# orybkin/video-gcp

Measured on AMD Instinct MI355X. Metric: predicted frames/sec, 64x64x3 seq_len=80 gcp_tree (posterior forward + all loss terms, model(inputs) and model.loss() of train.py:157-159, batch-stat BatchNorm), higher is better.
Workload: dtype f32 (encoder / decoder convs and the tree GEMMs from 512 rows: split-f16 MFMA with f32 accumulate, f32-equivalent; everything else exact f32 MFMA)

## Files before the change

### include/gcpx.h

```cpp
#ifndef GCPX_H
#define GCPX_H

#include <stdint.h>

#ifdef __cplusplus
extern "C" {
#endif

#define GCPX_VERSION 1

typedef enum gcpx_status {
    GCPX_OK = 0,
    GCPX_ERR_INVALID_ARG = -1,
    GCPX_ERR_UNSUPPORTED = -2,
    GCPX_ERR_HIP = -3,
    GCPX_ERR_COMM = -4
} gcpx_status;

typedef enum gcpx_act { GCPX_ACT_NONE = 0, GCPX_ACT_LRELU = 1, GCPX_ACT_TANH = 2 } gcpx_act;

int gcpx_version(void);
const char* gcpx_last_error(void);
int gcpx_conv_grid(void);

// ... 23 lines not shown
    int32_t Hin, Win;
    int32_t Hout, Wout;
    int32_t Cin;
    int32_t Cout;
    int32_t out_pitch;
    int32_t upsample;
    int32_t out_act;
    int32_t head_mode;
    const float* wpk;
    const float* bias;
    float* out;
    float* images;
    float* stats_partial;
    const int32_t* raw_row_map;
    const int32_t* src_row_map;
    const int32_t* src_row_frames;
    int32_t n_src_rows;
    int32_t w_split_log2;
    const void* wpk_split;
    const int32_t* w_split_log2_dev;
    int32_t split_layout;
    int32_t nll_rows;
    const float* nll_target;
    float* nll_partial;
    const float* nll_row_weight;
    float nll_scale;
    int32_t _pad3;
    float* images_rows;
    int64_t images_rows_dup;
    const float* bwd_r;
    const float *bwd_scale, *bwd_shift, *bwd_mean, *bwd_rstd;
    const float* addend;
    int32_t addend_frame_div;
    int32_t _pad4;
} gcpx_conv_args;

typedef enum gcpx_split_layout { GCPX_SPLIT_PLAIN = 0, GCPX_SPLIT_ROWFOLD = 1, GCPX_SPLIT_HEAD32 = 2, GCPX_SPLIT_ROWFOLD16 = 3,
                                 GCPX_SPLIT_LOWRES = 4 } gcpx_split_layout;

int gcpx_conv3x3(const gcpx_conv_args* a, void* stream);
int gcpx_conv3x3_grid(const gcpx_conv_args* a);
int gcpx_conv3x3_lowres_supported(const gcpx_conv_args* a);
int gcpx_conv4x4s2(const gcpx_conv_args* a, void* stream);
int gcpx_conv4x4s2_grid(void);
int gcpx_conv4x4s2_image(const float* x, const float* wpk, const float* bias, float* out,
                         int32_t F, int32_t Hin, int32_t Win, int32_t Cout, int32_t out_act, void* stream);

int gcpx_bn_finalize(const float* partial, int32_t n_partial, int32_t pitch, int32_t C, double count,
                     const float* gamma, const float* beta, float eps, float* scale, float* shift,
                     float* running_mean, float* running_var, float momentum, float* mean_out, float* rstd_out,
                     void* stream);
int gcpx_randn(float* out, int64_t n, uint64_t* state, void* stream);
int gcpx_bn_fold(const float* running_mean, const float* running_var, const float* gamma, const float* beta,
                 float eps, int32_t C, float* scale, float* shift, void* stream);

typedef struct gcpx_row_src {
    const float* ptr;
    const int32_t* rowidx;
    const float* scale;
    const float* shiftv;
    int64_t sb, sr;
    int32_t width;
    int32_t shift;
    int32_t act;
    int32_t cmod;
} gcpx_row_src;

typedef enum gcpx_gemm_epi {
    GCPX_EPI_NONE = 0,
    GCPX_EPI_LRELU = 1,
    GCPX_EPI_LSTM = 2,
    GCPX_EPI_GAUSS_SAMPLE = 3
} gcpx_gemm_epi;

struct gcpx_lstm_bwd_args;
// ... 552 lines not shown
```

### video-gcp_amd/csrc/conv3x3_split.hip

```cpp
#include "common.h"
#include "split_mfma.h"

#include <cstdlib>
#include <type_traits>

namespace {

struct SplitUpCfg {
    static constexpr int RW = 18, RH = 6, LW = 10, LH = 4, CC = 16, KS = 5;
    static constexpr int RAW_BYTES = LH * LW * CC * 4;
    static constexpr int PLANE_BYTES = RH * RW * 32;
    static constexpr int WAVE_BYTES = RAW_BYTES + 2 * PLANE_BYTES;
    static constexpr int NS = (LH * LW * 4 + 63) / 64;
    static constexpr int W_CHUNK_BYTES = KS * 2 * 1024;
    static int lds_bytes(int nchunk) { return nchunk * W_CHUNK_BYTES + 8 * WAVE_BYTES + 8 * 2 * 16 * 4; }
};

__global__ void __launch_bounds__(512, 2) conv3x3_up16_split_kernel(const gcpx_conv_args a, const int items_per_wave,
                                                                    const int nitems) {
    using Cfg = SplitUpCfg;
    constexpr int RW = Cfg::RW, RH = Cfg::RH, LW = Cfg::LW, LH = Cfg::LH, CC = Cfg::CC, NS = Cfg::NS, KS = Cfg::KS;
    extern __shared__ float4 smem4[];
    const int nchunk = a.Cin / CC;
    const char* wl = reinterpret_cast<const char*>(smem4);
// ... 1389 lines not shown

int gcpx_launch_up32_split(const gcpx_conv_args* a, hipStream_t stream, int which, int grid) {
    if (a->split_layout == GCPX_SPLIT_LOWRES) return gcpx_launch_lowres(a, stream, grid);
    if (which == 0) return launch_up32_split<2, 1>(a, stream, grid);
    if (which == 1) return launch_up32_split<2, 2>(a, stream, grid);
    return launch_up32_split<4, 2>(a, stream, grid);
}

int gcpx_launch_up16_fold(const gcpx_conv_args* a, hipStream_t stream, int grid) {
    using Cfg = FoldCfg;
    GCPX_CHECK_ARG(a->Cin == 32 && a->Cout == 16 && a->Hin % Cfg::R == 0 && a->Hout == 2 * a->Hin && a->Wout == 2 * a->Win && a->Wout % 16 == 0,
                   "row-folded block: 32 -> 16 channels, Hin a multiple of 4, output width a multiple of 16");
    GCPX_CHECK_ARG(a->src[0].C % 4 == 0 && (a->nsrc == 1 ? a->src[0].C == 32 : a->src[0].C + a->src[1].C == 32), "source channels");
    static const bool prio = getenv("GCPX_FOLD_NOPRIO") == nullptr;
    auto kern = prio ? conv3x3_up16_fold_kernel<true> : conv3x3_up16_fold_kernel<false>;
    static bool attr_set = false;
    if (!attr_set) {
        for (auto k : {conv3x3_up16_fold_kernel<true>, conv3x3_up16_fold_kernel<false>}) {
            hipError_t e = hipFuncSetAttribute(reinterpret_cast<const void*>(k), hipFuncAttributeMaxDynamicSharedMemorySize, Cfg::LDS_BYTES);
            if (e != hipSuccess) {
                gcpx_set_error("conv3x3 row-folded up16: hipFuncSetAttribute(%d B LDS): %s", Cfg::LDS_BYTES, hipGetErrorString(e));
                return GCPX_ERR_HIP;
            }
        }
        attr_set = true;
    }
    const int nitems = a->F * (a->Hin / Cfg::R) * (a->Wout / 16);
    const int ipw = (nitems + grid * 8 - 1) / (grid * 8);
    hipLaunchKernelGGL(kern, dim3(grid), dim3(512), Cfg::LDS_BYTES, stream, *a, ipw, nitems);
    GCPX_CHECK_LAUNCH();
    return GCPX_OK;
}

int gcpx_launch_up16_fold16(const gcpx_conv_args* a, hipStream_t stream, int grid) {
    using Cfg = Fold16Cfg;
    GCPX_CHECK_ARG(a->Cin == 16 && a->Cout == 16 && a->nsrc == 1 && a->src[0].C == 16 && a->Hin % Cfg::R == 0 && a->Hout == 2 * a->Hin &&
                   a->Wout == 2 * a->Win && a->Wout % 16 == 0,
                   "row-folded 16-channel block: one 16-channel source, 16 output channels, Hin a multiple of 4, output width a multiple of 16");
    GCPX_CHECK_ARG(!a->addend || (a->addend_frame_div > 0 && a->F % a->addend_frame_div == 0),
                   "row-folded 16-channel block: F must be a multiple of addend_frame_div (items are walked sequence by sequence)");
    auto kern = conv3x3_up16_fold16_kernel;
    static bool attr_set = false;
    if (!attr_set) {
        hipError_t e = hipFuncSetAttribute(reinterpret_cast<const void*>(kern), hipFuncAttributeMaxDynamicSharedMemorySize, Cfg::LDS_BYTES);
        if (e != hipSuccess) {
            gcpx_set_error("conv3x3 row-folded up16 (16 channels): hipFuncSetAttribute(%d B LDS): %s", Cfg::LDS_BYTES, hipGetErrorString(e));
            return GCPX_ERR_HIP;
        }
        attr_set = true;
    }
    const int nitems = a->F * (a->Hin / Cfg::R) * (a->Wout / 16);
    const int ipw = (nitems + grid * 8 - 1) / (grid * 8);
    hipLaunchKernelGGL(kern, dim3(grid), dim3(512), Cfg::LDS_BYTES, stream, *a, ipw, nitems);
    GCPX_CHECK_LAUNCH();
    return GCPX_OK;
}

extern "C" int gcpx_fold_upsample_weights(const float* w, int32_t Cout, int32_t Cin, float* out, void* stream_) {
    GCPX_CHECK_ARG(w && out && Cout > 0 && Cin > 0, "bad arguments");
    const int n = 24 * Cout * Cin;
    hipLaunchKernelGGL(fold_up_weights_kernel, dim3((n + 255) / 256), dim3(256), 0, reinterpret_cast<hipStream_t>(stream_), w, Cout, Cin, out);
    GCPX_CHECK_LAUNCH();
    return GCPX_OK;
}

int gcpx_launch_wave_split(const gcpx_conv_args* a, hipStream_t stream, int ct, int depth) {
    const int nchunk = a->Cin / 16;
    if (ct == 1) {
// ... 11 lines not shown
```

### video-gcp_amd/packing.py

```python
import torch

_LANE = torch.arange(64)
_LI = _LANE % 16
_LQ = _LANE // 16


def _pad_rows(w, rows):
    if w.shape[0] == rows:
        return w
    pad = torch.zeros((rows - w.shape[0],) + tuple(w.shape[1:]), dtype=w.dtype, device=w.device)
    return torch.cat([w, pad], 0)


def pack_gemm(w):
    N, K = w.shape
    assert K % 16 == 0, (N, K)
    NT = (N + 15) // 16
    w = _pad_rows(w, NT * 16)
    dev = w.device
    kg = torch.arange(K // 16, device=dev)[:, None, None, None]
    nt = torch.arange(NT, device=dev)[None, :, None, None]
    li = _LI.to(dev)[None, None, :, None]
    lq = _LQ.to(dev)[None, None, :, None]
    s = torch.arange(4, device=dev)[None, None, None, :]
# ... 236 lines not shown


def bilinear_x2_matrix(n, dtype=torch.float64):
    U = torch.zeros(2 * n, n, dtype=dtype)
    for h in range(2 * n):
        s = h // 2
        s0, s1, w0 = (s, min(s + 1, n - 1), 0.75) if h % 2 else (max(s - 1, 0), s, 0.25)
        U[h, s0] += w0
        U[h, s1] += 1.0 - w0
    return U


def lowres_up_reference(x, w, b):
    x, w = x.double(), w.double()
    Fr, _, H, W = x.shape
    cout = w.shape[0]
    Uy, Ux = bilinear_x2_matrix(H), bilinear_x2_matrix(W)
    out = torch.zeros(Fr, cout, 2 * H, 2 * W, dtype=torch.float64)
    for ty in range(3):
        z = torch.zeros(Fr, cout, H, 2 * W, dtype=torch.float64)
        for tx in range(3):
            y = torch.einsum("oc,fchw->fohw", w[:, :, ty, tx], x)
            yx = torch.einsum("fohw,pw->fohp", y, Ux)
            lo, hi = max(0, 1 - tx), min(2 * W, 2 * W + 1 - tx)
            z[..., lo:hi] += yx[..., lo + tx - 1:hi + tx - 1]
        zy = torch.einsum("qh,fohp->foqp", Uy, z)
        lo, hi = max(0, 1 - ty), min(2 * H, 2 * H + 1 - ty)
        out[:, :, lo:hi] += zy[:, :, lo + ty - 1:hi + ty - 1]
    if b is not None:
        out += b.double()[None, :, None, None]
    return out


def conv3x3_split32_index(shape, offset):
    n = 1
    for d in shape:
        n *= d
    ids = (torch.arange(n, dtype=torch.float64) + (offset + 1)).view(shape)
    return (conv3x3_split32_gather(ids).reshape(-1) - 1).to(torch.int32)


def head32_slot(c, i, n_mix=10):
    g, h, r = i // 8, (i // 4) % 2, i % 4
    if c < 3:
        m, p = 2 * c + g // 2, 4 * (g % 2) + r
        return 8 * (2 * m + h) + p if m < 5 else -1
    u = 4 * g + r
    return dlm_log_scale_slot(1 + u % 2, 2 * (u // 2) + h, n_mix) if u < 10 else -1


def head32_gather(w, perm):
    assert w.shape[1] == 16 and w.shape[0] == 100
    dev = w.device
    chan = torch.tensor([[perm[head32_slot(c, i)] if head32_slot(c, i) >= 0 else -1 for i in range(32)] for c in range(4)], device=dev)
    wz = torch.cat([w.reshape(100, 16, 9), torch.zeros((1, 16, 9), dtype=w.dtype, device=dev)], 0)
    chan = torch.where(chan >= 0, chan, torch.full_like(chan, 100))
    tap = torch.arange(9, device=dev)[:, None, None, None]
    ct = torch.arange(4, device=dev)[None, :, None, None]
    lane = torch.arange(64, device=dev)[None, None, :, None]
    el = torch.arange(8, device=dev)[None, None, None, :]
    return wz[chan[ct, lane % 32], (lane // 32) * 8 + el, tap].contiguous()


def pack_head32_split(w, perm):
    w1, w2, e = split_f16(head32_gather(w, perm))
    return torch.stack([w1, w2], 2).contiguous().view(torch.int16), e
# ... 39 lines not shown
def pack_conv3x3_fold(w):
    w1, w2, e = split_f16(conv3x3_fold_gather(fold_up_weights(w)))
    return torch.stack([w1, w2], 1).contiguous().view(torch.int16), e


def conv3x3_fold_index():
    ids = torch.arange(24 * 16 * 32, dtype=torch.float64).view(24, 16, 32)
    return conv3x3_fold_gather(ids).reshape(-1).to(torch.int32)


def conv3x3_fold16_gather(fw, cbase=0):
    assert fw.shape[0] == 24 and fw.shape[1] == 16 and fw.shape[2] >= cbase + 16
    dev = fw.device
    bases = [py * 9 + dyl * 3 for py in range(2) for dyl in range(3)] + [18, 21]
    fz = torch.cat([fw, torch.zeros((1,) + tuple(fw.shape[1:]), dtype=fw.dtype, device=dev)], 0)
    li, lq = _LI.to(dev)[:, None], _LQ.to(dev)[:, None]
    el = torch.arange(8, device=dev)[None, :]
    frags = []
    for b in bases:
        for kind in range(2):
            tset = (b + lq // 2) if kind == 0 else torch.where(lq // 2 == 0, torch.full_like(lq, b + 2), torch.full_like(lq, 24))
            frags.append(fz[tset, li, cbase + 8 * (lq % 2) + el])
    return torch.stack(frags, 0).contiguous()


def pack_conv3x3_fold16(w, cbase=0):
    w1, w2, e = split_f16(conv3x3_fold16_gather(fold_up_weights(w), cbase))
    return torch.stack([w1, w2], 1).contiguous().view(torch.int16), e


def conv3x3_fold16_index(cin, cbase):
    ids = (torch.arange(24 * 16 * cin, dtype=torch.float64) + 1).view(24, 16, cin)
    return (conv3x3_fold16_gather(ids, cbase).reshape(-1) - 1).to(torch.int32)


def lstm_gate_interleave(w_ih, w_hh, b_ih, b_hh):
    H = w_hh.shape[1]
    w = torch.cat([w_ih, w_hh], dim=1)
    K = w.shape[1]
    w = w.view(4, H, K).permute(1, 0, 2).reshape(4 * H, K)
    b = (b_ih + b_hh).view(4, H).t().reshape(4 * H)
    return w.contiguous(), b.contiguous()


def unpack_conv4x4(wpk, cin, cout):
    dev = wpk.device
    wpk = wpk.reshape(16, cin // 16, cout // 16, 64, 4)
    w = torch.zeros((cout, cin, 16), dtype=wpk.dtype, device=dev)
    tap = torch.arange(16, device=dev)[:, None, None, None, None]
    cg = torch.arange(cin // 16, device=dev)[None, :, None, None, None]
    ct = torch.arange(cout // 16, device=dev)[None, None, :, None, None]
    li = _LI.to(dev)[None, None, None, :, None]
    lq = _LQ.to(dev)[None, None, None, :, None]
    s = torch.arange(4, device=dev)[None, None, None, None, :]
    w[(ct * 16 + li).expand_as(wpk), (cg * 16 + lq * 4 + s).expand_as(wpk), tap.expand_as(wpk)] = wpk
    return w.reshape(cout, cin, 4, 4)


def encoder_frames_unsupported(hp):
    if hp.input_nc != 3:
        return f"input_nc = {hp.input_nc}: 3 is built"
    if hp.img_sz not in (32, 64):
        return f"img_sz = {hp.img_sz}: 32 and 64 are built"
    if hp.ngf != 16:
        return f"ngf = {hp.ngf}: 16 is built"
    if hp.nz_enc <= 0 or hp.nz_enc % 16 or hp.nz_enc > 256:
# ... 69 lines not shown
```

### video-gcp_amd/runtime.py

```python
import ctypes as C
import os

_HERE = os.path.dirname(os.path.abspath(__file__))
LIB_PATH = os.path.join(_HERE, "libgcpx.so")

ACT_NONE, ACT_LRELU, ACT_TANH = 0, 1, 2
HEAD_RAW, HEAD_DLM_MEAN, HEAD_DLM_BOTH, HEAD_TANH_NCHW, HEAD_DLM_NLL, HEAD_DLM_NLL_GRAD = 0, 1, 2, 3, 4, 5
SPLIT_PLAIN, SPLIT_ROWFOLD, SPLIT_HEAD32, SPLIT_ROWFOLD16, SPLIT_LOWRES = 0, 1, 2, 3, 4
EPI_NONE, EPI_LRELU, EPI_LSTM, EPI_GAUSS_SAMPLE = 0, 1, 2, 3
GEMM_FORM_TILE, GEMM_FORM_SPLIT_K, GEMM_FORM_SPLIT_F16, GEMM_FORM_PLANES = 0, 1, 2, 3
MLP_PLAIN, MLP_GAUSS, MLP_TANH = 0, 1, 2

vp = C.c_void_p
i32 = C.c_int32
i64 = C.c_int64


class ConvSrc(C.Structure):
    _fields_ = [("ptr", vp), ("scale", vp), ("shift", vp), ("C", i32), ("frame_div", i32), ("act", i32), ("_pad", i32)]


class ConvArgs(C.Structure):
    _fields_ = [("src", ConvSrc * 2), ("nsrc", i32), ("F", i32), ("Hin", i32), ("Win", i32), ("Hout", i32),
                ("Wout", i32), ("Cin", i32), ("Cout", i32), ("out_pitch", i32), ("upsample", i32), ("out_act", i32),
                ("head_mode", i32), ("wpk", vp), ("bias", vp), ("out", vp), ("images", vp), ("stats_partial", vp),
                ("raw_row_map", vp), ("src_row_map", vp), ("src_row_frames", vp), ("n_src_rows", i32), ("w_split_log2", i32), ("wpk_split", vp), ("w_split_log2_dev", vp),
                ("split_layout", i32), ("nll_rows", i32), ("nll_target", vp), ("nll_partial", vp), ("nll_row_weight", vp),
                ("nll_scale", C.c_float), ("_pad3", i32), ("images_rows", vp), ("images_rows_dup", i64), ("bwd_r", vp), ("bwd_scale", vp), ("bwd_shift", vp), ("bwd_mean", vp),
                ("bwd_rstd", vp), ("addend", vp), ("addend_frame_div", i32), ("_pad4", i32)]


class LossArgs(C.Structure):
    _fields_ = [("nll_bt", vp), ("pad_mask", vp), ("kl_b", vp), ("len_logits", vp), ("end_ind", vp), ("existence", vp),
                ("leave", vp), ("regressed_state", vp), ("state_target", vp), ("seq_len", vp), ("out", vp),
                ("B", i32), ("T", i32), ("N", i32), ("state_dim", i32), ("w_rec", C.c_float), ("w_kl", C.c_float),
                ("w_len", C.c_float), ("w_exist", C.c_float), ("w_state", C.c_float), ("total_div", C.c_float),
                ("action_pred", vp), ("action_seq", vp), ("inv_t0", vp), ("cost_pred", vp), ("cost_target", vp),
                ("n_actions", i32), ("w_action", C.c_float), ("w_cost", C.c_float), ("state_mask", vp), ("w_kl_dev", vp)]


class RowSrc(C.Structure):
    _fields_ = [("ptr", vp), ("rowidx", vp), ("scale", vp), ("shiftv", vp), ("sb", i64), ("sr", i64),
                ("width", i32), ("shift", i32), ("act", i32), ("cmod", i32)]


class GemmArgs(C.Structure):
    _fields_ = [("src", RowSrc * 6), ("nsrc", i32), ("M", i32), ("N", i32), ("K", i32), ("rpb", i32),
                ("wpk", vp), ("bias", vp), ("out", vp), ("ob", i64), ("orow", i64), ("epi", i32), ("nbatch", i32),
                ("stats_partial", vp), ("c_prev", vp), ("c_prev_stride", i64), ("h_out", vp), ("c_out", vp),
                ("hb", i64), ("hrow", i64), ("h_copy", vp), ("z_src_off", i64), ("z_w_off", i64),
                ("z_bias_off", i64), ("z_out_off", i64), ("gates_out", vp),
                ("wpk_split", vp), ("w_split_log2_dev", vp), ("w_split_log2", i32), ("_pad_split", i32),
                ("x_planes", vp), ("x_exp", vp), ("x_planes_bytes", i64), ("lstm_bwd", vp)]


class MlpArgs(C.Structure):
    _fields_ = [("src", RowSrc * 6), ("nsrc", i32), ("M", i32), ("rpb", i32), ("in_dim", i32), ("mid", i32),
                ("n_mid", i32), ("out_dim", i32), ("w_in", vp), ("b_in", vp), ("w_mid", vp), ("b_mid", vp),
                ("gn_gamma", vp), ("gn_beta", vp), ("w_out", vp), ("b_out", vp), ("gn_eps", C.c_float),
                ("lrelu_slope", C.c_float), ("epi", i32), ("out_split", i32), ("out", vp), ("ob", i64), ("orow", i64),
                ("oblk", i64), ("eps", vp), ("eb", i64), ("erow", i64), ("z", vp), ("zb", i64), ("zrow", i64), ("save", vp)]

# ... 40 lines not shown
class ActBwdArgs(C.Structure):
    _fields_ = [("da", vp), ("add", vp), ("r", vp), ("scale", vp), ("shift", vp), ("mean", vp), ("rstd", vp), ("dy", vp),
                ("stats_partial", vp), ("ldc", i64), ("c_off", i32), ("up", i32), ("fsum", i32), ("act", i32), ("F", i32),
                ("H", i32), ("W", i32), ("C", i32)]


class PanelTile(C.Structure):
    _fields_ = [("kind", i32), ("src", i32), ("index", i32), ("length", i32), ("flags", i32), ("nb", i32), ("nf", i32),
                ("h", i32), ("w", i32), ("tile_w", i32), ("n0", i32), ("n_b", i32), ("n_f", i32), ("r0", i32), ("r_b", i32),
                ("r_f", i32), ("c0", i32), ("c_b", i32), ("c_f", i32), ("index_off", i32), ("index_stride", i32),
                ("index_count", i32), ("fill", C.c_float), ("_pad", i32), ("off", i64), ("s_b", i64), ("s_f", i64), ("s_c", i64),
                ("s_y", i64)]


class TrajLayer(C.Structure):
    _fields_ = [("states", vp), ("s_n", i64), ("s_p", i64), ("s_d", i64), ("len", vp), ("dim_t", vp), ("color", C.c_float * 3),
                ("len_i64", i32), ("K", i32), ("P", i32)]


PANEL_MAX_SRCS = 16
PANEL_IMAGE, PANEL_GREY, PANEL_GREY_ADD, PANEL_FILL = 0, 1, 2, 3
PANEL_RESCALE, PANEL_LENGTH_STRICT, PANEL_INDEX_FRAME, PANEL_INDEX_I64, PANEL_LENGTH_I64 = 1, 2, 4, 8, 16

WG_ROWS, WG_CONV1D, WG_CONV3X3, WG_CONV4X4S2 = 0, 1, 2, 3
WMAP_LINEAR, WMAP_CONV, WMAP_CONVT = 0, 1, 2

SYMBOLS = [
    ("gcpx_version", C.c_int, []),
    ("gcpx_last_error", C.c_char_p, []),
    ("gcpx_conv_grid", C.c_int, []),
    ("gcpx_conv3x3", C.c_int, [C.POINTER(ConvArgs), vp]),
    ("gcpx_conv3x3_grid", C.c_int, [C.POINTER(ConvArgs)]),
    ("gcpx_conv3x3_lowres_supported", C.c_int, [C.POINTER(ConvArgs)]),
    ("gcpx_conv4x4s2", C.c_int, [C.POINTER(ConvArgs), vp]),
    ("gcpx_conv4x4s2_grid", C.c_int, []),
    ("gcpx_conv4x4s2_image", C.c_int, [vp, vp, vp, vp, i32, i32, i32, i32, i32, vp]),
    ("gcpx_bn_finalize", C.c_int, [vp, i32, i32, i32, C.c_double, vp, vp, C.c_float, vp, vp, vp, vp, C.c_float, vp, vp, vp]),
    ("gcpx_bn_fold", C.c_int, [vp, vp, vp, vp, C.c_float, i32, vp, vp, vp]),
    ("gcpx_randn", C.c_int, [vp, i64, vp, vp]),
    ("gcpx_gemm", C.c_int, [C.POINTER(GemmArgs), vp]),
    ("gcpx_gemm_row_blocks", C.c_int, [i32, i32]),
    ("gcpx_gemm_form", C.c_int, [C.POINTER(GemmArgs), vp]),
    ("gcpx_gemm_planes_workspace", C.c_int, [i32, i32, i32, vp, vp]),
    ("gcpx_mlp", C.c_int, [C.POINTER(MlpArgs), vp]),
    ("gcpx_balanced_binding", C.c_int, [vp, i32, i32, i32, vp, vp, vp, vp, vp, vp, vp]),
    ("gcpx_dlm_nll", C.c_int, [vp, vp, vp, vp, i32, i32, i32, i32, vp]),
    ("gcpx_gauss_nll", C.c_int, [vp, vp, vp, vp, i32, i32, vp]),
    ("gcpx_kl_gauss", C.c_int, [vp, vp, i32, i32, i32, i64, i64, C.c_float, vp, i64, vp, vp]),
    ("gcpx_gauss_sample", C.c_int, [vp, i64, i64, vp, i64, i64, vp, i64, i64, i32, i32, i32, vp]),
    ("gcpx_seq_index", C.c_int, [vp, i32, i32, vp, vp, vp]),
    ("gcpx_fill_zero", C.c_int, [vp, i64, vp]),
    ("gcpx_copy_rows", C.c_int, [vp, vp, i32, i32, i64, i64, i64, vp]),
    ("gcpx_loss_combine", C.c_int, [C.POINTER(LossArgs), vp]),
    ("gcpx_loss_pre", C.c_int, [C.POINTER(LossArgs), vp, vp, i32, i32, i64, i64, C.c_float, vp, i64, vp, vp]),
    ("gcpx_loss_final", C.c_int, [C.POINTER(LossArgs), vp]),
    ("gcpx_gather_rows", C.c_int, [vp, vp, vp, i32, i32, i32, i32, i64, vp]),
    ("gcpx_gather_rows_rest", C.c_int, [vp, vp, vp, i32, i32, i32, i32, i64, vp, vp]),
    ("gcpx_compact_index", C.c_int, [vp, i32, i32, i32, vp, vp]),
    ("gcpx_seq_pairs", C.c_int, [vp, vp, vp, vp, i32, i32, i32, vp]),
    ("gcpx_rollout_cost", C.c_int, [vp, i64, vp, vp, i64, vp, i32, i32, i32, i32, i32, C.c_float, vp]),
    ("gcpx_masked_row_sum", C.c_int, [vp, vp, vp, i32, i32, vp]),
    ("gcpx_wgrad", C.c_int, [C.POINTER(WgradArgs), vp]),
    ("gcpx_wgrad_classify", C.c_int, [C.POINTER(WgradArgs), i32, C.POINTER(C.c_int32), C.POINTER(C.c_int32)]),
    ("gcpx_wgrad_group", C.c_int, [vp, vp, i32, i32, i32, vp]),
    ("gcpx_wgrad_conv3x3", C.c_int, [vp, i32, vp, i32, i32, i32, i32, i32, vp, i32, vp]),
    ("gcpx_wgrad_conv3x3_split", C.c_int, [vp, i32, vp, i32, i32, i32, i32, i32, vp, i32, vp]),
# ... 164 lines not shown
```

### video-gcp_amd/weights.py

```python
import ctypes as C
import os
from contextlib import contextmanager

import torch

from . import packing as pk
from . import runtime as rt
from .hparams import GCPHParams
from .params import init_params, encoder_layers, encoder_skip_layers, decoder_layers
from .plan_ops import _addr


class WeightsMixin:

    def _flatten_params(self, params):
        off, self._poff = 0, {}
        for k, v in params.items():
            self._poff[k] = (off, tuple(v.shape))
            off += (v.numel() + 3) // 4 * 4
        self.theta = torch.zeros(off, dtype=torch.float32, device=self.device)
        self.sd = {}
        for k, v in params.items():
            o, shp = self._poff[k]
            view = self.theta[o:o + v.numel()].view(shp)
            view.copy_(v)
            self.sd[k] = view

    def _pack_predictor(self, prefix, out_dim):
        sd = self._psd
        mid = sd[f"{prefix}.input.linear.weight"].shape[0]
        n_mid = 0
        while f"{prefix}.pyramid-{n_mid}.linear.weight" in sd:
            n_mid += 1
        out_pad = (out_dim + 15) // 16 * 16
        w_in = sd[f"{prefix}.input.linear.weight"]
        k_raw = w_in.shape[1]
        if k_raw % 16:
            w_in = torch.cat([w_in, torch.zeros((mid, -k_raw % 16), dtype=w_in.dtype, device=w_in.device)], 1)
        d = dict(mid=mid, n_mid=n_mid, out_dim=out_dim, in_dim=w_in.shape[1], in_dim_raw=k_raw)
        d["w_in"] = pk.pack_gemm(w_in)
        d["b_in"] = sd[f"{prefix}.input.linear.bias"].contiguous()
        if n_mid:
            d["w_mid"] = torch.stack([pk.pack_gemm(sd[f"{prefix}.pyramid-{i}.linear.weight"]) for i in range(n_mid)]).contiguous()
# ... 29 lines not shown
                if self.split_f16 and skip_idx >= 0 and c_prev == 16 and c_skip == 16 and os.environ.get("GCPX_NO_SKIP_HOIST") is None:
                    hoist16.add(f"dec.{name}")
            elif cout == 16:
                todo.append((f"dec.{name}", f"decoder.net.{name}.conv.weight", None))
            elif cout in (32, 64) and (c_prev + c_skip) % 32 == 0:
                todo.append((f"dec.{name}", f"decoder.net.{name}.conv.weight", "tiled32"))
        for name, cin, cout, norm in self._enc_layers[1:]:
            if cin == 16 or cin % 32 == 0:
                todo.append((f"enc.{name}", f"encoder.net.{name}.conv.weight", "enc4x4"))
        for name, key, perm in todo:
            off, shp = self._poff[key]
            d = {}
            if perm == "enc4x4":
                idx = pk.conv4x4_split_index(shp, off).to(self.device)
            elif perm == "rowfold":
                d["fold"] = torch.zeros(24 * shp[0] * shp[1], dtype=torch.float32, device=self.device)
                d["fold_src"] = (off, shp[0], shp[1])
                idx = pk.conv3x3_fold_index().to(self.device)
            elif perm == "tiled32":
                idx = pk.conv3x3_split32_index(shp, off).to(self.device)
            elif isinstance(perm, tuple) and perm[0] == "head32":
                idx = pk.head32_index(shp, off, perm[1]).to(self.device)
            else:
                idx = pk.conv3x3_split_index(shp, off, perm).to(self.device)
            d.update(idx=idx, out=torch.zeros(2 * idx.numel(), dtype=torch.int16, device=self.device),
                     log2=torch.zeros(1, dtype=torch.int32, device=self.device))
            self.pk_split[name] = d
            if perm == "rowfold" and name in hoist16:
                for tag, cbase in (("f16a", 0), ("f16b", 16)):
                    i16 = pk.conv3x3_fold16_index(shp[1], cbase).to(self.device)
                    self.pk_split[f"{name}.{tag}"] = dict(fold=d["fold"], fold16=True, idx=i16,
                                                          out=torch.zeros(2 * i16.numel(), dtype=torch.int16, device=self.device),
                                                          log2=torch.zeros(1, dtype=torch.int32, device=self.device))
        self.repack_split()

    def repack_split(self, stream=None):
        st = stream if stream is not None else torch.cuda.current_stream(self.device).cuda_stream
        if not self.pk_split:
            return
        tab = self._split_tab
        key = (self.theta.data_ptr(),) + tuple((d["out"].data_ptr(), d["idx"].data_ptr()) for d in self.pk_split.values())
        if tab is None or tab[2] != key:
            descs = []
            for name, d in self.pk_split.items():
                src = d["fold"] if "fold" in d else self.theta
                e = rt.SplitPackDesc()
                e.src, e.idx, e.out, e.log2_out, e.n = src.data_ptr(), d["idx"].data_ptr(), d["out"].data_ptr(), d["log2"].data_ptr(), d["idx"].numel()
                descs.append(e)
            arr = (rt.SplitPackDesc * len(descs))(*descs)
            dev = torch.frombuffer(bytearray(bytes(arr)), dtype=torch.uint8).to(self.device)
            tab = self._split_tab = (dev, len(descs), key, torch.zeros(len(descs), dtype=torch.int32, device=self.device))
        for name, d in self.pk_split.items():
            if "fold_src" in d:
                off, cout, cin = d["fold_src"]
                rt.check(self.lib.gcpx_fold_upsample_weights(self.theta.data_ptr() + 4 * off, cout, cin, d["fold"].data_ptr(), st), "fold_upsample_weights")
        rt.check(self.lib.gcpx_split_pack_group2(tab[0].data_ptr(), tab[1], tab[3].data_ptr(), st), "split_pack_group2")

    def _pack_gemm_split(self):
        self._gsplit = {}
        self._merge_side_rows = int(os.environ.get("GCPX_MERGE_SIDE_ROWS", "512")) or (1 << 60)
        pr = int(os.environ.get("GCPX_GEMM_PLANES_ROWS", "512"))
        self._planes_min_rows = pr if pr > 0 else 1 << 60
        if not self.split_f16:
            return
        for name, W in self.pk.items():
            if not (isinstance(W, dict) and name.startswith("tree")):
                continue
            for key, wpk in W.items():
                if not (key.endswith(".w") and (key.startswith("lstm") or key == "proj.w")):
                    continue
                stack = wpk if wpk.dim() == 5 else wpk[None]
                if (stack.shape[2] * 16) % 64 or (stack.shape[1] * 16) % 64:
                    continue
                packs = [pk.pack_gemm_split(pk.unpack_gemm(w, w.shape[1] * 16)) for w in stack]
                ws = torch.stack([p_[0] for p_ in packs]).contiguous().to(self.device)
                es = torch.tensor([p_[1] for p_ in packs], dtype=torch.int32, device=self.device)
                self._gsplit[wpk.data_ptr()] = (ws, es)

    def _set_split(self, a, name):
        d = self.pk_split.get(name)
        layout = None
        if name == "dec.head" and self.head32 and a.head_mode in (rt.HEAD_DLM_MEAN, rt.HEAD_DLM_NLL, rt.HEAD_DLM_NLL_GRAD) \
                and "dec.head32" in self.pk_split:
            d, layout = self.pk_split["dec.head32"], rt.SPLIT_HEAD32
        if self.split_f16 and d is not None:
            a.wpk_split, a.w_split_log2_dev = d["out"].data_ptr(), d["log2"].data_ptr()
            if layout is None:
                layout = rt.SPLIT_ROWFOLD16 if d.get("fold16") else (rt.SPLIT_ROWFOLD if "fold" in d else rt.SPLIT_PLAIN)
            a.split_layout = layout
            if layout == rt.SPLIT_PLAIN and os.environ.get("GCPX_NO_LOWRES") is None and \
                    self.lib.gcpx_conv3x3_lowres_supported(C.byref(a)):
                a.split_layout = rt.SPLIT_LOWRES

    def _pack_fused_embed(self):
        hp = self._hp
        for l in range(hp.hierarchy_levels if hp.untied_layers else 1):
            p = f"tree_module.tree_modules.{l}.subgoal_pred"
            sd = self.sd
            We, be = sd[f"{p}.embed.weight"].double(), sd[f"{p}.embed.bias"].double()
            Wih = sd[f"{p}.lstm.0.weight_ih"].double()
            Wf = (Wih @ We).float()
            bf = (Wih @ be).float() + sd[f"{p}.lstm.0.bias_ih"]
            w, b = pk.lstm_gate_interleave(Wf, sd[f"{p}.lstm.0.weight_hh"], bf, sd[f"{p}.lstm.0.bias_hh"])
            self.pk[f"tree{l}"]["lstm0f.w"], self.pk[f"tree{l}"]["lstm0f.b"] = pk.pack_gemm(w), b

    def _pack_tree(self, sd):
        hp = self._hp
        self._psd = sd
        P = {}
        layers, c_top = encoder_layers(hp)
        self._enc_layers, self._c_top = layers, c_top
        P["enc.input.w"] = pk.pack_conv4x4_image(sd["encoder.net.input.conv.weight"])
        P["enc.input.b"] = sd["encoder.net.input.conv.bias"].contiguous()
        for name, cin, cout, norm in layers[1:]:
            P[f"enc.{name}.w"] = pk.pack_conv4x4(sd[f"encoder.net.{name}.conv.weight"])
            P[f"enc.{name}.b"] = sd[f"encoder.net.{name}.conv.bias"].contiguous()
        wh = sd["encoder.net.head.weight"]
        P["enc.head.w"] = pk.pack_gemm(wh.permute(0, 2, 3, 1).reshape(hp.nz_enc, 16 * c_top))
        P["enc.head.b"] = sd["encoder.net.head.bias"].contiguous()
        wt = sd["decoder.net.input.conv.weight"]
        P["dec.input.w"] = pk.pack_gemm(wt.permute(2, 3, 1, 0).reshape(16 * c_top, hp.nz_enc))
        P["dec.input.b"] = sd["decoder.net.input.conv.bias"].repeat(16).contiguous()
# ... 202 lines not shown
```

Baseline: 507,800.

## Add column-form up16 conv3x3 kernel computing upsample via post-conv horizontal interpolation

Adds a new kernel for the 16-channel bilinear-upsample-then-conv3x3 decoder block. It folds the vertical upsample into the weights and convolves at input column resolution. The horizontal x2 interpolation is then applied to the three column-tap outputs using DPP lane shifts, so the MFMA work scales with input width rather than output width. A new weight packing and an up16_form switch route the first-half channel block to this kernel by default. The cost is more complex boundary handling and changed f16-split rounding order, plus LDS sized for one block per CU.

After: 511,000 (median of 6 runs). Within noise of the previous version (+0.6%).

```diff
diff --git a/include/gcpx.h b/include/gcpx.h
--- a/include/gcpx.h
+++ b/include/gcpx.h
@@ -79,7 +79,7 @@
     const float *bwd_scale, *bwd_shift, *bwd_mean, *bwd_rstd;
     const float* addend;
     int32_t addend_frame_div;
-    int32_t _pad4;
+    int32_t up16_form;
 } gcpx_conv_args;
 
 typedef enum gcpx_split_layout { GCPX_SPLIT_PLAIN = 0, GCPX_SPLIT_ROWFOLD = 1, GCPX_SPLIT_HEAD32 = 2, GCPX_SPLIT_ROWFOLD16 = 3,
@@ -88,6 +88,7 @@
 int gcpx_conv3x3(const gcpx_conv_args* a, void* stream);
 int gcpx_conv3x3_grid(const gcpx_conv_args* a);
 int gcpx_conv3x3_lowres_supported(const gcpx_conv_args* a);
+int gcpx_conv3x3_up16_cols_supported(const gcpx_conv_args* a);
 int gcpx_conv4x4s2(const gcpx_conv_args* a, void* stream);
 int gcpx_conv4x4s2_grid(void);
 int gcpx_conv4x4s2_image(const float* x, const float* wpk, const float* bias, float* out,
diff --git a/video-gcp_amd/csrc/conv3x3_split.hip b/video-gcp_amd/csrc/conv3x3_split.hip
--- a/video-gcp_amd/csrc/conv3x3_split.hip
+++ b/video-gcp_amd/csrc/conv3x3_split.hip
@@ -1445,8 +1445,12 @@
     return GCPX_OK;
 }
 
+int gcpx_launch_up16_cols(const gcpx_conv_args* a, hipStream_t stream, int grid);
+
 int gcpx_launch_up16_fold16(const gcpx_conv_args* a, hipStream_t stream, int grid) {
     using Cfg = Fold16Cfg;
+    GCPX_CHECK_ARG(a->up16_form == 0 || a->up16_form == 1, "up16_form: 0 (conv3x3_fold16 pack) or 1 (conv3x3_cols16 pack)");
+    if (a->up16_form == 1) return gcpx_launch_up16_cols(a, stream, grid);
     GCPX_CHECK_ARG(a->Cin == 16 && a->Cout == 16 && a->nsrc == 1 && a->src[0].C == 16 && a->Hin % Cfg::R == 0 && a->Hout == 2 * a->Hin &&
                    a->Wout == 2 * a->Win && a->Wout % 16 == 0,
                    "row-folded 16-channel block: one 16-channel source, 16 output channels, Hin a multiple of 4, output width a multiple of 16");
diff --git a/video-gcp_amd/csrc/conv3x3_up16_cols.hip b/video-gcp_amd/csrc/conv3x3_up16_cols.hip
--- /dev/null
+++ b/video-gcp_amd/csrc/conv3x3_up16_cols.hip
@@ -0,0 +1,317 @@
+#include "common.h"
+#include "split_mfma.h"
+
+#include <type_traits>
+
+namespace {
+
+template <int TILES>
+struct ColsCfg {
+    static constexpr int R = 2, SR = R + 2, WIN = 16 * TILES;
+    static constexpr int PLANE_BYTES = SR * WIN * 32;
+    static constexpr int WAVE_BYTES = 2 * PLANE_BYTES;
+    static constexpr int NT = 18;
+    static constexpr int W_BYTES = NT * 2048;
+    static constexpr int LDS_BYTES = W_BYTES + 8 * WAVE_BYTES + 8 * 2 * 16 * 4 + 3 * 16 * 4;
+    static constexpr int NS = SR * WIN * 4 / 64;
+};
+
+template <int CTRL>
+__device__ __forceinline__ float dpp_keep(const float old, const float v) {
+    return __int_as_float(__builtin_amdgcn_update_dpp(__float_as_int(old), __float_as_int(v), CTRL, 0xf, 0xf, false));
+}
+
+template <int TILES>
+__global__ void __launch_bounds__(512, 1) conv3x3_up16_cols_kernel(const gcpx_conv_args a, const int items_per_wave, const int nitems) {
+    using Cfg = ColsCfg<TILES>;
+    constexpr int R = Cfg::R, SR = Cfg::SR, WIN = Cfg::WIN, NS = Cfg::NS;
+    extern __shared__ float4 smem4[];
+    const char* wl = reinterpret_cast<const char*>(smem4);
+    const int tid = threadIdx.x, lane = tid & 63;
+    const int wave = __builtin_amdgcn_readfirstlane(tid >> 6);
+    char* wbuf = reinterpret_cast<char*>(smem4) + Cfg::W_BYTES + wave * Cfg::WAVE_BYTES;
+    float* red = reinterpret_cast<float*>(reinterpret_cast<char*>(smem4) + Cfg::W_BYTES + 8 * Cfg::WAVE_BYTES);
+    float* biasl = red + 8 * 2 * 16;
+    const int j = lane & 15, q = lane >> 4;
+    const int H = a.Hout, W = a.Wout, Hin = a.Hin;
+    const int nrb = Hin / R;
+
+    for (int i = tid; i < Cfg::W_BYTES / 16; i += 512) smem4[i] = reinterpret_cast<const float4*>(a.wpk_split)[i];
+    if (tid < 16) {
+        biasl[tid] = a.bias[tid];
+        biasl[16 + tid] = a.src[0].scale ? a.src[0].scale[tid] : 1.f;
+        biasl[32 + tid] = a.src[0].scale ? a.src[0].shift[tid] : 0.f;
+    }
+    __syncthreads();
+
+    const int c4 = lane & 3, ps = lane >> 2;
+    const float* sptr = a.src[0].ptr;
+    const float slope = a.src[0].act == GCPX_ACT_LRELU ? 0.2f : 1.f;
+    const int fdiv0 = a.src[0].frame_div;
+    const int ew = a.w_split_log2_dev ? __builtin_amdgcn_readfirstlane(*a.w_split_log2_dev) : a.w_split_log2;
+    const float4 bv = *reinterpret_cast<const float4*>(a.bias + q * 4);
+
+    const int gw = blockIdx.x * 8 + wave;
+    const int item0 = gw * items_per_wave;
+    const int item_end = min(item0 + items_per_wave, nitems);
+    const float* const addend = a.addend;
+    const int div = addend ? a.addend_frame_div : 1;
+    auto origin = [&](int it, int& run, int& f, int& y0) {
+        run = it / div;
+        const int rb = run % nrb;
+        y0 = rb * R;
+        f = (run / nrb) * div + (it - run * div);
+    };
+    float4 pre[NS];
+    auto issue_loads = [&](int it) __attribute__((always_inline)) {
+        int run, f, y0;
+        origin(it, run, f, y0);
+        const float* base = sptr + (size_t)(f / fdiv0) * Hin * WIN * 16;
+#pragma unroll
+        for (int k = 0; k < NS; ++k) {
+            const int sy = min(max(y0 - 1 + k / TILES, 0), Hin - 1);
+            pre[k] = *reinterpret_cast<const float4*>(base + (unsigned)((sy * WIN + (k % TILES) * 16 + ps) * 16 + c4 * 4));
+        }
+    };
+    const int st_wr = ps * 32 + c4 * 8;
+    const int boff0 = ((q >> 1) * WIN + j) * 32 + (q & 1) * 16, boff1 = j * 32 + (q & 1) * 16;
+
+    const float kl75 = j == 0 ? 0.f : 0.75f, kl25 = j == 0 ? 0.f : 0.25f;
+    const float kr75 = j == 15 ? 0.f : 0.75f, kr25 = j == 15 ? 0.f : 0.25f;
+
+    f32x4 ab[R][2][TILES][2];
+#pragma unroll
+    for (int yi = 0; yi < R; ++yi)
+#pragma unroll
+        for (int py = 0; py < 2; ++py)
+#pragma unroll
+            for (int t = 0; t < TILES; ++t) { ab[yi][py][t][0] = f32x4{bv.x, bv.y, bv.z, bv.w}; ab[yi][py][t][1] = ab[yi][py][t][0]; }
+    int ab_run = -1;
+
+    f32x4 st1 = f32x4{0, 0, 0, 0}, st2 = f32x4{0, 0, 0, 0};
+    if (item0 < item_end) issue_loads(item0);
+    __builtin_amdgcn_s_waitcnt(0x0f70);
+
+    for (int item = item0; item < item_end; ++item) {
+        int run, f, y0;
+        origin(item, run, f, y0);
+        const bool top = (y0 == 0), bot = (y0 + R == Hin);
+        const unsigned lane_out = (unsigned)(2 * j * 16 + q * 4);
+        const bool odd = j & 1;
+        const unsigned line_out = (unsigned)((j & ~1) * 32 + (j & 1) * 16 + q * 4);
+
+        if (addend && run != ab_run) {
+            ab_run = run;
+            const float* adp = addend + ((size_t)(f / div) * H + 2 * y0) * W * 16;
+            const float4 bl = *reinterpret_cast<const float4*>(biasl + q * 4);
+#pragma unroll
+            for (int yi = 0; yi < R; ++yi)
+#pragma unroll
+                for (int py = 0; py < 2; ++py)
+#pragma unroll
+                    for (int t = 0; t < TILES; ++t)
+#pragma unroll
+                        for (int eo = 0; eo < 2; ++eo) {
+                            const float4 ad = *reinterpret_cast<const float4*>(adp + (unsigned)((2 * yi + py) * W * 16 + (t * 32 + eo) * 16) + lane_out);
+                            ab[yi][py][t][eo] = f32x4{ad.x + bl.x, ad.y + bl.y, ad.z + bl.z, ad.w + bl.w};
+                        }
+        }
+
+        float amax = 0.f;
+        const float4 bn_s = *reinterpret_cast<const float4*>(biasl + 16 + c4 * 4), bn_t = *reinterpret_cast<const float4*>(biasl + 32 + c4 * 4);
+#pragma unroll
+        for (int k = 0; k < NS; ++k) {
+            float4 v = pre[k];
+            v.x = fmaf(v.x, bn_s.x, bn_t.x); v.y = fmaf(v.y, bn_s.y, bn_t.y); v.z = fmaf(v.z, bn_s.z, bn_t.z); v.w = fmaf(v.w, bn_s.w, bn_t.w);
+            v.x = fmaxf(v.x, v.x * slope); v.y = fmaxf(v.y, v.y * slope); v.z = fmaxf(v.z, v.z * slope); v.w = fmaxf(v.w, v.w * slope);
+            pre[k] = v;
+            amax = vmax3abs(amax, v.x, v.y);
+            amax = vmax3abs(amax, v.z, v.w);
+        }
+        amax = wave_max_nonneg(amax);
+        int ex = 14 + 127 - (int)((__float_as_uint(amax) >> 23) & 0xff);
+        ex = __builtin_amdgcn_readfirstlane(amax > 0.f ? max(-100, min(min(100, 126 - ew), ex)) : min(100, 126 - ew));
+        const float sx2 = __uint_as_float((unsigned)(127 + ex) << 23);
+#pragma unroll
+        for (int k = 0; k < NS; ++k) {
+            h4 p1, p2;
+            split4(pre[k], sx2, p1, p2);
+            *reinterpret_cast<h4*>(wbuf + st_wr + k * 512) = p1;
+            *reinterpret_cast<h4*>(wbuf + st_wr + k * 512 + Cfg::PLANE_BYTES) = p2;
+        }
+        issue_loads(min(item + 1, item_end - 1));
+        __builtin_amdgcn_fence(__ATOMIC_ACQ_REL, "wavefront");
+        __builtin_amdgcn_wave_barrier();
+
+        auto load_w = [&](const int t, h8 (&w)[2]) __attribute__((always_inline)) {
+            const char* wp = wl + t * 2048 + lane * 16;
+            w[0] = *reinterpret_cast<const h8*>(wp);
+            w[1] = *reinterpret_cast<const h8*>(wp + 1024);
+        };
+        auto load_b = [&](const int ks, const int yi, h8 (&b)[TILES][2]) __attribute__((always_inline)) {
+#pragma unroll
+            for (int t = 0; t < TILES; ++t) {
+                const char* bp = wbuf + (ks ? boff1 + (yi + 2) * WIN * 32 : boff0 + yi * WIN * 32) + t * 512;
+                b[t][0] = *reinterpret_cast<const h8*>(bp);
+                b[t][1] = *reinterpret_cast<const h8*>(bp + Cfg::PLANE_BYTES);
+            }
+        };
+
+        const float inv = __uint_as_float((unsigned)(127 - ex - ew) << 23);
+        float* optr = a.out + ((size_t)f * H + 2 * y0) * W * 16;
+
+        h8 b0[TILES][2], b1[TILES][2];
+        static_for<0, 2 * R>([&](auto pc) __attribute__((always_inline)) {
+            constexpr int yi = decltype(pc)::value / 2, py = decltype(pc)::value % 2;
+            f32x4 acc[TILES][3];
+#pragma unroll
+            for (int t = 0; t < TILES; ++t)
+#pragma unroll
+                for (int tx = 0; tx < 3; ++tx) acc[t][tx] = f32x4{0, 0, 0, 0};
+            h8 wq[2][2], wc[2];
+            load_w(py * 6, wq[0]);
+            if constexpr (py == 0) { load_b(0, yi, b0); load_b(1, yi, b1); }
+            __builtin_amdgcn_s_setprio(1);
+            static_for<0, 6>([&](auto bc) __attribute__((always_inline)) {
+                constexpr int blk = decltype(bc)::value, ks = blk / 3, tx = blk % 3;
+                constexpr bool more = blk + 1 < 6;
+                if constexpr (more) load_w(py * 6 + ((blk + 1) % 3) * 2 + (blk + 1) / 3, wq[(blk + 1) & 1]);
+                auto& bq = *(ks ? &b1 : &b0);
+                const h8 w1 = wq[blk & 1][0], w2 = wq[blk & 1][1];
+#pragma unroll
+                for (int t = 0; t < TILES; ++t) acc[t][tx] = mfma32h(w2, bq[t][0], acc[t][tx]);
+#pragma unroll
+                for (int t = 0; t < TILES; ++t) acc[t][tx] = mfma32h(w1, bq[t][1], acc[t][tx]);
+#pragma unroll
+                for (int t = 0; t < TILES; ++t) acc[t][tx] = mfma32h(w1, bq[t][0], acc[t][tx]);
+                __builtin_amdgcn_sched_group_barrier(0x100, more ? 2 : 0, 0);
+                __builtin_amdgcn_sched_group_barrier(0x008, 3 * TILES, 0);
+            });
+            if constexpr ((yi == 0 && py == 0) || (yi == R - 1 && py == 1)) {
+                if (py == 0 ? top : bot) {
+                    auto& bc = *(py ? &b1 : &b0);
+#pragma unroll
+                    for (int tx = 0; tx < 3; ++tx) {
+                        load_w(12 + py * 3 + tx, wc);
+#pragma unroll
+                        for (int t = 0; t < TILES; ++t) {
+                            acc[t][tx] = mfma32h(wc[1], bc[t][0], acc[t][tx]);
+                            acc[t][tx] = mfma32h(wc[0], bc[t][1], acc[t][tx]);
+                            acc[t][tx] = mfma32h(wc[0], bc[t][0], acc[t][tx]);
+                        }
+                    }
+                }
+            }
+            __builtin_amdgcn_s_setprio(0);
+
+#pragma unroll
+            for (int t = 0; t < TILES; ++t) {
+                const float cl75 = t == 0 ? kl75 : 0.75f, cl25 = t == 0 ? kl25 : 0.25f;
+                const float cr75 = t == TILES - 1 ? kr75 : 0.75f, cr25 = t == TILES - 1 ? kr25 : 0.25f;
+                f32x4 ve, vo;
+#pragma unroll
+                for (int r = 0; r < 4; ++r) {
+                    const float y0v = acc[t][0][r], y1v = acc[t][1][r], y2v = acc[t][2][r];
+                    float el0 = y0v, el1 = y1v, er1 = y1v, er2 = y2v;
+                    if (t > 0) {
+                        el0 = dpp_keep<0x121>(0.f, acc[t > 0 ? t - 1 : 0][0][r]);
+                        el1 = dpp_keep<0x121>(0.f, acc[t > 0 ? t - 1 : 0][1][r]);
+                    }
+                    if (t + 1 < TILES) {
+                        er1 = dpp_keep<0x12F>(0.f, acc[t + 1 < TILES ? t + 1 : t][1][r]);
+                        er2 = dpp_keep<0x12F>(0.f, acc[t + 1 < TILES ? t + 1 : t][2][r]);
+                    }
+                    const float p0 = dpp_keep<0x111>(el0, y0v), p1 = dpp_keep<0x111>(el1, y1v);
+                    const float n1 = dpp_keep<0x101>(er1, y1v), n2 = dpp_keep<0x101>(er2, y2v);
+                    float e = cl75 * p0;
+                    e = fmaf(cl25, y0v, e); e = fmaf(0.25f, p1, e); e = fmaf(0.75f, y1v, e); e = fmaf(0.75f, y2v, e); e = fmaf(0.25f, n2, e);
+                    float o = 0.25f * p0;
+                    o = fmaf(0.75f, y0v, o); o = fmaf(0.75f, y1v, o); o = fmaf(0.25f, n1, o); o = fmaf(cr25, y2v, o); o = fmaf(cr75, n2, o);
+                    ve[r] = fmaf(e, inv, ab[yi][py][t][0][r]);
+                    vo[r] = fmaf(o, inv, ab[yi][py][t][1][r]);
+                }
+                f32x4 s1, s2;
+#pragma unroll
+                for (int r = 0; r < 4; ++r) {
+                    const float give = odd ? ve[r] : vo[r];
+                    const float take = dpp_keep<0xB1>(0.f, give);
+                    s1[r] = odd ? take : ve[r];
+                    s2[r] = odd ? vo[r] : take;
+                }
+                float* ob = optr + (unsigned)((2 * yi + py) * W * 16 + t * 32 * 16) + line_out;
+                __builtin_nontemporal_store(s1, reinterpret_cast<f32x4*>(ob));
+                __builtin_nontemporal_store(s2, reinterpret_cast<f32x4*>(ob + 32));
+#pragma unroll
+                for (int r = 0; r < 4; ++r) {
+                    st1[r] += ve[r]; st2[r] = fmaf(ve[r], ve[r], st2[r]);
+                    st1[r] += vo[r]; st2[r] = fmaf(vo[r], vo[r], st2[r]);
+                }
+            }
+        });
+        __builtin_amdgcn_fence(__ATOMIC_ACQ_REL, "wavefront");
+        __builtin_amdgcn_wave_barrier();
+    }
+    if (a.stats_partial) {
+#pragma unroll
+        for (int r = 0; r < 4; ++r) {
+            const float s1 = row16_sum(st1[r]);
+            const float s2 = row16_sum(st2[r]);
+            if (j == 0) {
+                red[(wave * 2 + 0) * 16 + q * 4 + r] = s1;
+                red[(wave * 2 + 1) * 16 + q * 4 + r] = s2;
+            }
+        }
+        __syncthreads();
+        if (tid < 32) {
+            const int which = tid >> 4, c = tid & 15;
+            float sum = 0.f;
+#pragma unroll
+            for (int w = 0; w < 8; ++w) sum += red[(w * 2 + which) * 16 + c];
+            a.stats_partial[((size_t)blockIdx.x * 2 + which) * 16 + c] = sum;
+        }
+    }
+}
+
+int cols_tiles(const gcpx_conv_args* a) {
+    if (!a || !a->upsample || !a->wpk_split || !a->out || !a->bias) return 0;
+    if (a->head_mode != GCPX_HEAD_RAW || a->out_act != GCPX_ACT_NONE || a->out_pitch != 16) return 0;
+    if (a->src_row_map || a->raw_row_map || a->bwd_r) return 0;
+    if (a->Cin != 16 || a->Cout != 16 || a->nsrc != 1 || !a->src[0].ptr || a->src[0].C != 16 || a->src[0].frame_div <= 0) return 0;
+    if (a->F <= 0 || a->Hin <= 0 || a->Hin % 2 || a->Hout != 2 * a->Hin || a->Wout != 2 * a->Win) return 0;
+    if (a->addend && (a->addend_frame_div <= 0 || a->F % a->addend_frame_div)) return 0;
+    return a->Win == 16 ? 1 : a->Win == 32 ? 2 : 0;
+}
+
+template <int TILES>
+int launch_cols(const gcpx_conv_args* a, hipStream_t stream, int grid) {
+    using Cfg = ColsCfg<TILES>;
+    auto kern = conv3x3_up16_cols_kernel<TILES>;
+    static bool attr_set = false;
+    if (!attr_set) {
+        hipError_t e = hipFuncSetAttribute(reinterpret_cast<const void*>(kern), hipFuncAttributeMaxDynamicSharedMemorySize, Cfg::LDS_BYTES);
+        if (e != hipSuccess) {
+            gcpx_set_error("conv3x3 up16 column form: hipFuncSetAttribute(%d B LDS): %s", Cfg::LDS_BYTES, hipGetErrorString(e));
+            return GCPX_ERR_HIP;
+        }
+        attr_set = true;
+    }
+    const int nitems = a->F * (a->Hin / Cfg::R);
+    const int ipw = (nitems + grid * 8 - 1) / (grid * 8);
+    hipLaunchKernelGGL(kern, dim3(grid), dim3(512), Cfg::LDS_BYTES, stream, *a, ipw, nitems);
+    GCPX_CHECK_LAUNCH();
+    return GCPX_OK;
+}
+
+}
+
+extern "C" int gcpx_conv3x3_up16_cols_supported(const gcpx_conv_args* a) { return cols_tiles(a) > 0 ? 1 : 0; }
+
+int gcpx_launch_up16_cols(const gcpx_conv_args* a, hipStream_t stream, int grid) {
+    switch (cols_tiles(a)) {
+        case 1: return launch_cols<1>(a, stream, grid);
+        case 2: return launch_cols<2>(a, stream, grid);
+    }
+    gcpx_set_error("conv3x3 up16 column form: up16_form = 1 on a problem gcpx_conv3x3_up16_cols_supported refuses (Cin=%d Cout=%d Hin=%d Win=%d)",
+                   a->Cin, a->Cout, a->Hin, a->Win);
+    return GCPX_ERR_UNSUPPORTED;
+}
diff --git a/video-gcp_amd/packing.py b/video-gcp_amd/packing.py
--- a/video-gcp_amd/packing.py
+++ b/video-gcp_amd/packing.py
@@ -292,6 +292,38 @@
     return out
 
 
+def up16_cols_reference(x, w, b):
+    x, w = x.double(), w.double()
+    Fr, _, H, W = x.shape
+    cout = w.shape[0]
+    rows = [x[:, :, [min(max(y - 1 + d, 0), H - 1) for y in range(H)]] for d in range(3)]
+    out = torch.zeros(Fr, cout, 2 * H, 2 * W, dtype=torch.float64)
+    cm = [max(c - 1, 0) for c in range(W)]
+    cp = [min(c + 1, W - 1) for c in range(W)]
+    for py in range(2):
+        Y = []
+        for tx in range(3):
+            y = torch.zeros(Fr, cout, H, W, dtype=torch.float64)
+            for dyl in range(3):
+                c = _FOLD_CF[py][dyl]
+                fw = c[0] * w[:, :, 0, tx] + c[1] * w[:, :, 1, tx] + c[2] * w[:, :, 2, tx]
+                y += torch.einsum("oc,fchw->fohw", fw, rows[dyl])
+            if py == 0:
+                y[:, :, 0] -= torch.einsum("oc,fcw->fow", w[:, :, 0, tx], x[:, :, 0])
+            else:
+                y[:, :, H - 1] -= torch.einsum("oc,fcw->fow", w[:, :, 2, tx], x[:, :, H - 1])
+            Y.append(y)
+        e0 = 0.75 * Y[0][..., cm] + 0.25 * Y[0]
+        e0[..., 0] = 0.0
+        o2 = 0.25 * Y[2] + 0.75 * Y[2][..., cp]
+        o2[..., W - 1] = 0.0
+        out[:, :, py::2, 0::2] = e0 + (0.25 * Y[1][..., cm] + 0.75 * Y[1]) + (0.75 * Y[2] + 0.25 * Y[2][..., cp])
+        out[:, :, py::2, 1::2] = (0.25 * Y[0][..., cm] + 0.75 * Y[0]) + (0.75 * Y[1] + 0.25 * Y[1][..., cp]) + o2
+    if b is not None:
+        out += b.double()[None, :, None, None]
+    return out
+
+
 def conv3x3_split32_index(shape, offset):
     n = 1
     for d in shape:
@@ -397,6 +429,31 @@
 def conv3x3_fold16_index(cin, cbase):
     ids = (torch.arange(24 * 16 * cin, dtype=torch.float64) + 1).view(24, 16, cin)
     return (conv3x3_fold16_gather(ids, cbase).reshape(-1) - 1).to(torch.int32)
+
+
+def conv3x3_cols16_gather(fw, cbase=0):
+    assert fw.shape[0] == 24 and fw.shape[1] == 16 and fw.shape[2] >= cbase + 16
+    dev = fw.device
+    fz = torch.cat([fw, torch.zeros((1,) + tuple(fw.shape[1:]), dtype=fw.dtype, device=dev)], 0)
+    li, lq = _LI.to(dev)[:, None], _LQ.to(dev)[:, None]
+    el = torch.arange(8, device=dev)[None, :]
+    half = lambda t: torch.where(lq // 2 == 0, torch.full_like(lq, t), torch.full_like(lq, 24))
+    sets = []
+    for py in range(2):
+        for tx in range(3):
+            sets += [py * 9 + 3 * (lq // 2) + tx, half(py * 9 + 6 + tx)]
+    sets += [half(18 + tx) for tx in range(3)] + [half(21 + tx) for tx in range(3)]
+    return torch.stack([fz[t, li, cbase + 8 * (lq % 2) + el] for t in sets], 0).contiguous()
+
+
+def pack_conv3x3_cols16(w, cbase=0):
+    w1, w2, e = split_f16(conv3x3_cols16_gather(fold_up_weights(w), cbase))
+    return torch.stack([w1, w2], 1).contiguous().view(torch.int16), e
+
+
+def conv3x3_cols16_index(cin, cbase):
+    ids = (torch.arange(24 * 16 * cin, dtype=torch.float64) + 1).view(24, 16, cin)
+    return (conv3x3_cols16_gather(ids, cbase).reshape(-1) - 1).to(torch.int32)
 
 
 def lstm_gate_interleave(w_ih, w_hh, b_ih, b_hh):
diff --git a/video-gcp_amd/runtime.py b/video-gcp_amd/runtime.py
--- a/video-gcp_amd/runtime.py
+++ b/video-gcp_amd/runtime.py
@@ -27,7 +27,7 @@
                 ("raw_row_map", vp), ("src_row_map", vp), ("src_row_frames", vp), ("n_src_rows", i32), ("w_split_log2", i32), ("wpk_split", vp), ("w_split_log2_dev", vp),
                 ("split_layout", i32), ("nll_rows", i32), ("nll_target", vp), ("nll_partial", vp), ("nll_row_weight", vp),
                 ("nll_scale", C.c_float), ("_pad3", i32), ("images_rows", vp), ("images_rows_dup", i64), ("bwd_r", vp), ("bwd_scale", vp), ("bwd_shift", vp), ("bwd_mean", vp),
-                ("bwd_rstd", vp), ("addend", vp), ("addend_frame_div", i32), ("_pad4", i32)]
+                ("bwd_rstd", vp), ("addend", vp), ("addend_frame_div", i32), ("up16_form", i32)]
 
 
 class LossArgs(C.Structure):
@@ -134,6 +134,7 @@
     ("gcpx_conv3x3", C.c_int, [C.POINTER(ConvArgs), vp]),
     ("gcpx_conv3x3_grid", C.c_int, [C.POINTER(ConvArgs)]),
     ("gcpx_conv3x3_lowres_supported", C.c_int, [C.POINTER(ConvArgs)]),
+    ("gcpx_conv3x3_up16_cols_supported", C.c_int, [C.POINTER(ConvArgs)]),
     ("gcpx_conv4x4s2", C.c_int, [C.POINTER(ConvArgs), vp]),
     ("gcpx_conv4x4s2_grid", C.c_int, []),
     ("gcpx_conv4x4s2_image", C.c_int, [vp, vp, vp, vp, i32, i32, i32, i32, i32, vp]),
diff --git a/video-gcp_amd/weights.py b/video-gcp_amd/weights.py
--- a/video-gcp_amd/weights.py
+++ b/video-gcp_amd/weights.py
@@ -9,6 +9,8 @@
 from .hparams import GCPHParams
 from .params import init_params, encoder_layers, encoder_skip_layers, decoder_layers
 from .plan_ops import _addr
+
+_UP16_COLS_TAGS = ("f16a",)
 
 
 class WeightsMixin:
@@ -104,6 +106,11 @@
                     self.pk_split[f"{name}.{tag}"] = dict(fold=d["fold"], fold16=True, idx=i16,
                                                           out=torch.zeros(2 * i16.numel(), dtype=torch.int16, device=self.device),
                                                           log2=torch.zeros(1, dtype=torch.int32, device=self.device))
+                    if tag in _UP16_COLS_TAGS:
+                        ic = pk.conv3x3_cols16_index(shp[1], cbase).to(self.device)
+                        self.pk_split[f"{name}.{tag}.cols"] = dict(fold=d["fold"], fold16=True, idx=ic,
+                                                                   out=torch.zeros(2 * ic.numel(), dtype=torch.int16, device=self.device),
+                                                                   log2=torch.zeros(1, dtype=torch.int32, device=self.device))
         self.repack_split()
 
     def repack_split(self, stream=None):
@@ -160,6 +167,10 @@
             if layout is None:
                 layout = rt.SPLIT_ROWFOLD16 if d.get("fold16") else (rt.SPLIT_ROWFOLD if "fold" in d else rt.SPLIT_PLAIN)
             a.split_layout = layout
+            dc = self.pk_split.get(name + ".cols")
+            if layout == rt.SPLIT_ROWFOLD16 and dc is not None and os.environ.get("GCPX_NO_UP16_COLS") is None and \
+                    self.lib.gcpx_conv3x3_up16_cols_supported(C.byref(a)):
+                a.wpk_split, a.w_split_log2_dev, a.up16_form = dc["out"].data_ptr(), dc["log2"].data_ptr(), 1
             if layout == rt.SPLIT_PLAIN and os.environ.get("GCPX_NO_LOWRES") is None and \
                     self.lib.gcpx_conv3x3_lowres_supported(C.byref(a)):
                 a.split_layout = rt.SPLIT_LOWRES
```
